# AnimatedRNG/alphazero-rs

Hardware: AMD Instinct MI355X
Metric: selfplay_games_per_sec (higher is better)
Workload: dtype bf16

## Files before the change

alphazero-rs_amd/csrc/az_engine.hip:

```cpp
#include "../../include/az_engine.h"

#include <dlfcn.h>
#include <unistd.h>
#include <rccl/rccl.h>

#include <algorithm>
#include <array>
#include <atomic>
#include <chrono>
#include <cstdio>
#include <cstring>
#include <map>
#include <memory>
#include <mutex>
#include <string>
#include <vector>

#include "az_combine.h"
#include "az_local_comm.h"
#include "az_net.h"
#include "az_train.h"
#include "az_tree.h"

using namespace az;
// ... 767 lines not shown
        return AZ_ERR_HIP;
    }
    *out = e.release();
    return AZ_OK;
}

void az_destroy(az_engine* e) {
    if (!e) return;
    (void)hipSetDevice(e->device);
    (void)hipStreamSynchronize(e->stream);
    (void)az_selfplay_end(e);
    for (auto& kv : e->nets) if (kv.second.conv) convnet_destroy(kv.second.conv);
    for (NetWorkspace* w : e->ws) netws_destroy(w);
    if (e->cache_keys) (void)hipFree(e->cache_keys);
    if (e->cache_pv) (void)hipFree(e->cache_pv);
    if (e->comm && g_rccl.CommDestroy) { (void)g_rccl.CommDestroy(e->comm); e->comm = nullptr; }
    if (e->local) { e->local->leave(e->comm_rank); e->local.reset(); }
    e->tree_pool.clear();
    trainer_destroy(e->trainer);
    { double ms[RG_COUNT] = {0, 0}; e->prof.resolve(ms); }
    (void)hipStreamDestroy(e->stream);
    delete e;
}

const char* az_last_error(const az_engine* e) { return e ? e->err.c_str() : "null engine"; }

az_status az_set_option(az_engine* e, const char* key, int64_t value) {
    if (!e || !key) return AZ_ERR_BAD_ARGUMENT;
    auto is = [&](const char* k) { return std::strcmp(key, k) == 0; };
    if (is("conv2_table") && (value == 0 || value == 1)) { e->netopt.conv2_table = (int)value; return AZ_OK; }
    if (is("conv3_small") && (value == 0 || value == 1)) { e->netopt.conv3_small = (int)value; return AZ_OK; }
    if (is("conv3_tail") && (value == 0 || value == 1)) { e->netopt.conv3_tail = (int)value; return AZ_OK; }
    if (is("ring_packed") && (value == 0 || value == 1)) { e->netopt.ring_packed = (int)value; return AZ_OK; }
    if (is("conv3_planes") && (value == 0 || value == 1)) { e->netopt.conv3_planes = (int)value; return AZ_OK; }
    if (is("narrow_rows") && value >= 0 && value <= 65536) { e->netopt.narrow_rows = (int)value; return AZ_OK; }
    if (is("tree_block4") && (value == 0 || value == 1)) { e->tree_block4 = (int)value; return AZ_OK; }
    if (is("dedup_stats") && (value == 0 || value == 1)) { e->dedup_stats = (int)value; return AZ_OK; }
    if (is("profile_every") && value >= 1 && value <= 1000000) { e->profile_every = (int)value; return AZ_OK; }
    if (is("profile") && (value == 0 || value == 1)) { e->prof.on = value != 0; return AZ_OK; }
    if (is("search_graph") && value >= 0 && value <= 1000 && value % 2 == 0) { e->search_graph = (int)value; return AZ_OK; }
    if (is("search_graph_rows") && value >= 0 && value <= 1000000) { e->search_graph_rows = (int)value; return AZ_OK; }
    if (is("selfplay_async") && (value == 0 || value == 1)) { e->selfplay_async = (int)value; return AZ_OK; }
    if (is("selfplay_async_launches") && value >= 1 && value <= 8) { e->selfplay_async_launches = (int)value; return AZ_OK; }
    if (is("selfplay_async_iters") && value >= 2 && value <= 64) { e->selfplay_async_iters = (int)value; return AZ_OK; }
    if (is("fused_search") && (value == 0 || value == 1)) { e->fused_search = (int)value; return AZ_OK; }
    if (is("eval_dedup") && value >= 0 && value <= 2) { e->eval_dedup = (int)value; return AZ_OK; }
    if (is("eval_cache_log2") && (value == 0 || (value >= 10 && value <= 30))) { e->eval_cache_log2 = (int)value; return AZ_OK; }
    if (is("eval_cache_max_stones") && value >= 0 && value <= 42) { e->eval_cache_max_stones = (int)value; return AZ_OK; }
    if (is("eval_cache_persist") && (value == 0 || value == 1)) { e->eval_cache_persist = (int)value; return AZ_OK; }
    if (is("train_epochs") && value >= 1 && value <= 100000) { e->train_epochs = (int)value; return AZ_OK; }
    if (is("train_batch") && value >= 2 && value <= TRAIN_MAX_BATCH) { e->train_batch = (int)value; return AZ_OK; }
    if (is("train_seed")) { e->train_seed = (uint64_t)value; return AZ_OK; }
    if (is("train_graph") && (value == 0 || value == 1)) { e->train_graph = (int)value; if (e->trainer) trainer_set_graph(e->trainer, value != 0); return AZ_OK; }
    if (is("train_gemm3_ring") && (value == 0 || value == 1)) { e->train_gemm3_ring = (int)value; if (e->trainer) trainer_set_gemm3_ring(e->trainer, value != 0); return AZ_OK; }
    if (is("train_fwd_x3") && (value == 0 || value == 1)) { e->train_fwd_x3 = (int)value; if (e->trainer) trainer_set_fwd_x3(e->trainer, value != 0); return AZ_OK; }
    if (is("train_wgrad_tr") && (value == 0 || value == 1)) { e->train_wgrad_tr = (int)value; if (e->trainer) trainer_set_wgrad_tr(e->trainer, value != 0); return AZ_OK; }
    if (is("train_implicit") && (value == 0 || value == 1)) { e->train_implicit = (int)value; if (e->trainer) trainer_set_implicit(e->trainer, value != 0); return AZ_OK; }
    if (is("train_fork") && (value == 0 || value == 1)) {
        e->train_fork = (int)value;
        if (e->trainer) { (void)hipSetDevice(e->device); trainer_set_fork(e->trainer, value != 0); }
        return AZ_OK;
    }
    if (is("train_gemm") && (value == 0 || value == 1)) { e->train_gemm = (int)value; if (e->trainer) trainer_set_gemm(e->trainer, (int)value); return AZ_OK; }
    if (is("train_fwd_dma") && (value == 0 || value == 1)) { e->train_fwd_dma = (int)value; if (e->trainer) trainer_set_fwd_dma(e->trainer, value != 0); return AZ_OK; }
    if (is("train_lr_e9") && value > 0) { e->hyper.lr = (float)((double)value * 1e-9); return AZ_OK; }
    if (is("train_dropout_e6") && value >= 0 && value < 1000000) { e->hyper.dropout = (float)((double)value * 1e-6); return AZ_OK; }
// ... 1425 lines not shown
```

alphazero-rs_amd/csrc/az_net.h:

```cpp
#pragma once
#include "az_tree.h"

namespace az {

struct ConvNet;
struct NetWorkspace;

struct Layout {
    int C;
    int64_t conv_w[4], conv_b[4], conv_bn[4], fc_w[2], fc_b[2], fc_bn[2], pi_w, pi_b, v_w, v_b, total;
    explicit Layout(int c) : C(c) {
        int64_t o = 0;
        for (int l = 0; l < 4; ++l) {
            int cin = l == 0 ? 2 : C;
            conv_w[l] = o; o += 9ll * cin * C;
            conv_b[l] = o; o += C;
            conv_bn[l] = o; o += 4ll * C;
        }
        const int fin[2] = {6 * C, 1024}, fout[2] = {1024, 512};
        for (int l = 0; l < 2; ++l) {
            fc_w[l] = o; o += (int64_t)fin[l] * fout[l];
            fc_b[l] = o; o += fout[l];
            fc_bn[l] = o; o += 4ll * fout[l];
        }
        pi_w = o; o += 512 * 7; pi_b = o; o += 7;
        v_w = o; o += 512; v_b = o; o += 1;
        total = o;
    }
};


struct NetProfile {
    double conv2_ms = 0, conv2_flops = 0, total_ms = 0, total_flops = 0;
    double conv3_ms = 0, conv3_flops = 0;
    double conv4_ms = 0, conv4_flops = 0;
    double fc_ms = 0, fc_flops = 0;
    double rows = 0;
    double conv2_bytes = 0;
    uint64_t launches = 0;
};

void launch_net_fixture(const EvalBatch& eb, int kind, uint64_t salt, hipStream_t s);

ConvNet* convnet_create(int channels, const char** err);
void convnet_destroy(ConvNet* n);
NetWorkspace* netws_create(int channels, int max_batch, const char** err);
void netws_destroy(NetWorkspace* ws);
int64_t convnet_param_count(int channels);
bool convnet_set_params(ConvNet* n, const float* host_params, int64_t count);
bool convnet_get_params(const ConvNet* n, float* host_params, int64_t count);
void convnet_init_random(ConvNet* n, uint64_t seed);
void netws_resolve_profile(NetWorkspace* ws, NetProfile* prof);
bool netws_conv3_accounting(NetWorkspace* ws, unsigned long long out[2], bool reset);
struct NetOptions {
    int conv2_table = 1;
    int conv3_small = 1;
    int conv3_planes = 1;
    int ring_packed = 1;
    int conv3_tail = 1;
    int narrow_rows = 32;
    int conv3_pp = 0;
    int gemm_variant = 5;
    int conv1_table = 1;
    int conv2_pipe = 1;
    int conv3_pipe = 1;
    int conv3_ring = 0;
    int conv4_big = 0;
    int fc_ring = 1;
    int ring_tile[6] = {0, 0, 0, 0, 0, 0};
};
bool netws_read_clock_stamps(NetWorkspace* ws, unsigned long long* out2048);
bool convnet_prepare(NetWorkspace* ws, const NetOptions& opt);
void convnet_forward(ConvNet* n, NetWorkspace* ws, const EvalBatch& eb, int n_rows_hint, int n_rows_typ, hipStream_t s, NetProfile* prof,
                     const NetOptions& opt);

}
```

alphazero-rs_amd/csrc/az_net.hip:

```cpp
#include "az_net.h"

#include <algorithm>
#include <cmath>
#include <cstring>
#include <vector>

namespace az {

constexpr int ACTIONS = ConnectFour::ACTIONS;

typedef __bf16 bf16x8 __attribute__((ext_vector_type(8)));
typedef float f32x4 __attribute__((ext_vector_type(4)));

__global__ void k_net_fixture(EvalBatch eb, int kind, uint64_t salt) {
    uint32_t i = blockIdx.x * blockDim.x + threadIdx.x;
    if (i >= *eb.n) return;
    float pi[ACTIONS], v;
    if (kind == 0) {
#pragma unroll
        for (int a = 0; a < ACTIONS; ++a) pi[a] = __fdiv_rn(1.0f, 7.0f);
        v = 1.0f;
    } else {
        ulonglong2 s = eb.state[i];
        hashnet_eval(s.x, s.y, salt, pi, &v);
// ... 161 lines not shown
                uint4 o;
                o.x = pack_bf16x2(fmaxf(acc[0] + b0.x, 0.f), fmaxf(acc[1] + b0.y, 0.f));
                o.y = pack_bf16x2(fmaxf(acc[2] + b0.z, 0.f), fmaxf(acc[3] + b0.w, 0.f));
                o.z = pack_bf16x2(fmaxf(acc[4] + b1.x, 0.f), fmaxf(acc[5] + b1.y, 0.f));
                o.w = pack_bf16x2(fmaxf(acc[6] + b1.z, 0.f), fmaxf(acc[7] + b1.w, 0.f));
                *(uint4*)(out + ((size_t)b * 42 + (size_t)(y * 7 + x)) * C + coff) = o;
            }
        }
    }
}

struct GemmDesc {
    const uint16_t* A;
    const uint16_t* W;
    const float* bias;
    uint16_t* out;
    const uint32_t* n_dev;
    int rows_per_sample;
    int out_w;
    int in_h, in_w, in_c;
    int tap_w;
    int cin;
    int K, N;
    int relu;
    unsigned long long* dbg;
    const ulonglong2* states;
    int out_f16;
    int m_min;
    int m_max;
    int m_hi;
    unsigned long long* acct;
    const uint16_t* c3tab;
    const uint16_t* Wp;
    const uint16_t* Wr;
};

constexpr int GBM = 128, GBN = 128, GBK = 64;

template <int LAYER>
__global__ __launch_bounds__(256, 2) void k_gemm_mfma(const GemmDesc d) {
    __shared__ __attribute__((aligned(16))) unsigned char smem[2][(GBM + GBN) * 128];
    const int M = (int)(*d.n_dev) * d.rows_per_sample;
    const int ntaps = d.K / d.cin;
    const int NT = d.N / GBN;
    const int id = blockIdx.x;
    const int xcd = id & 7, j = id >> 3;
    const int ntile = j % NT, mtile = (j / NT) * 8 + xcd;
    const int m0 = mtile * GBM, n0 = ntile * GBN;
    if (m0 >= M) return;
    const int tid = threadIdx.x, lane = tid & 63, wave = tid >> 6;
    const int wr = wave >> 1, wc = wave & 1;
    const int srow = tid >> 3;
    const int chunk = (tid & 7) ^ (srow & 7);
    auto row_off = [&](int q) -> uint32_t {
        int m = m0 + q * 32 + srow;
        m = m < M ? m : M - 1;
        const int b = m / d.rows_per_sample, r = m - b * d.rows_per_sample;
        const int y = r / d.out_w, x = r - y * d.out_w;
        return (uint32_t)(((b * d.in_h + y) * d.in_w + x) * d.in_c + chunk * 8);
    };
    const uint32_t a_off0 = row_off(0), a_off1 = row_off(1), a_off2 = row_off(2), a_off3 = row_off(3);
    const uint32_t b_off0 = (uint32_t)((n0 + srow) * d.K + chunk * 8), b_off1 = b_off0 + 32u * (uint32_t)d.K,
                   b_off2 = b_off0 + 64u * (uint32_t)d.K, b_off3 = b_off0 + 96u * (uint32_t)d.K;
    uint4 ra0, ra1, ra2, ra3, rb0, rb1, rb2, rb3;
#define AZ_GLOAD(kt_)                                                                           \
    {                                                                                           \
// ... 45 lines not shown
        if (kt + 1 < nk) AZ_SWRITE((kt + 1) & 1);
        __syncthreads();
    }
#undef AZ_GLOAD
#undef AZ_SWRITE
#pragma unroll
    for (int nt = 0; nt < 4; ++nt) {
        const int n = n0 + wc * 64 + nt * 16 + fq * 4;
        const float4 bv = d.out_f16 ? make_float4(0.f, 0.f, 0.f, 0.f) : *(const float4*)(d.bias + n);
#pragma unroll
        for (int mt = 0; mt < 4; ++mt) {
            const int m = m0 + wr * 64 + mt * 16 + frow;
            if (m >= M) continue;
            float r0 = acc[mt][nt][0] + bv.x, r1 = acc[mt][nt][1] + bv.y, r2 = acc[mt][nt][2] + bv.z,
                  r3 = acc[mt][nt][3] + bv.w;
            if (d.relu) { r0 = fmaxf(r0, 0.f); r1 = fmaxf(r1, 0.f); r2 = fmaxf(r2, 0.f); r3 = fmaxf(r3, 0.f); }
            uint2 o;
            if (d.out_f16) {
                o.x = pack_f16x2(r0, r1);
                o.y = pack_f16x2(r2, r3);
            } else {
                o.x = pack_bf16x2(r0, r1);
                o.y = pack_bf16x2(r2, r3);
            }
            *(uint2*)(d.out + (size_t)m * d.N + n) = o;
        }
    }
}

__device__ __forceinline__ void lds_dma16(const void* sbase , uint32_t voff, uint32_t lds_addr ) {
    asm volatile("s_mov_b32 m0, %2\n\ts_nop 0\n\tglobal_load_lds_dwordx4 %0, %1" ::"v"(voff), "s"(sbase), "s"(lds_addr) : "memory");
}

template <int NS, int BM>
__device__ __forceinline__ void gemm_ring_body(const GemmDesc& d, unsigned char* smem , const int M) {
    static_assert(BM % 32 == 0 && BM >= 64 && BM <= 192 && NS * (BM * 128 + 16384) <= 163840 && 2 * (BM / 32 + 4) <= 63, "tile");
    constexpr int MT = BM / 32;
    constexpr int STAGE = BM * 128 + 16384;
    constexpr int NDMA = MT + 4;
    const int ntaps = d.K / d.cin;
    const int NT = d.N / GBN;
    const int id = blockIdx.x;
    const int xcd = id & 7, j = id >> 3;
    const int ntile = j % NT, mtile = (j / NT) * 8 + xcd;
    const int m0 = mtile * BM, n0 = ntile * GBN;
    if (m0 >= M) return;
    const int tid = threadIdx.x, lane = tid & 63;
    const int wave = __builtin_amdgcn_readfirstlane(tid >> 6);
    const int wr = wave >> 1, wc = wave & 1;
    const int lrow = lane >> 3;
    const int chunk = (lane & 7) ^ lrow;
    uint32_t a_ob[MT];
#pragma unroll
    for (int q = 0; q < MT; ++q) {
        int m = m0 + (q * 4 + wave) * 8 + lrow;
        m = m < M ? m : M - 1;
        const int b = m / d.rows_per_sample, r = m - b * d.rows_per_sample;
        const int y = r / d.out_w, x = r - y * d.out_w;
        a_ob[q] = (uint32_t)(((b * d.in_h + y) * d.in_w + x) * d.in_c + chunk * 8) * 2u;
    }
    const bool packed = d.Wr != nullptr;
    const uint32_t b_ob = packed ? (uint32_t)(wave * 1024 + lane * 16)
                                 : (uint32_t)((n0 + wave * 8 + lrow) * d.K + chunk * 8) * 2u;
    const size_t w_stride = packed ? (size_t)4096 : (size_t)64 * d.K;
    const char* wr_tile = (const char*)d.Wr + (size_t)ntile * (size_t)(d.K / GBK) * 16384;
    int ks_idx = 0;
    typedef __attribute__((address_space(3))) void* lds_ptr;
    const uint32_t lds0 = (uint32_t)(uintptr_t)(lds_ptr)(smem + wave * 1024);
    int ks_tap = 0, ks_kx = 0;
    uint32_t ks_c0 = 0, ks_toff = 0, ks_kk = 0;
#define AZ_RDMA(buf_)                                                                                   \
    {                                                                                                   \
        const char* abase = (const char*)(d.A + ks_toff);                                               \
        const char* wbase = packed ? wr_tile + (size_t)ks_idx * 16384 : (const char*)(d.W + ks_kk);     \
        ++ks_idx;                                                                                       \
        const uint32_t la = lds0 + (buf_) * STAGE;                                                      \
        _Pragma("unroll") for (int q_ = 0; q_ < MT; ++q_) lds_dma16(abase, a_ob[q_], la + q_ * 4096);   \
        _Pragma("unroll") for (int q_ = 0; q_ < 4; ++q_) lds_dma16(wbase + q_ * w_stride, b_ob, la + BM * 128 + q_ * 4096); \
        ++ks_tap; ++ks_kx; ks_toff += (uint32_t)d.in_c; ks_kk += (uint32_t)d.cin;                       \
        if (ks_kx == d.tap_w) { ks_kx = 0; ks_toff += (uint32_t)((d.in_w - d.tap_w) * d.in_c); }        \
        if (ks_tap == ntaps) { ks_tap = 0; ks_kx = 0; ks_c0 += GBK; ks_toff = ks_c0; ks_kk = ks_c0; }   \
    }
    f32x4 acc[MT][4];
#pragma unroll
    for (int i = 0; i < MT; ++i)
#pragma unroll
        for (int jn = 0; jn < 4; ++jn) acc[i][jn] = f32x4{0.f, 0.f, 0.f, 0.f};
    const int nk = d.K / GBK;
    const int frow = lane & 15, fq = lane >> 4, fsw = lane & 7;
#pragma unroll
    for (int st = 0; st < NS - 1; ++st)
        if (st < nk) AZ_RDMA(st);
    for (int kt = 0; kt < nk; ++kt) {
        const int younger = nk - 1 - kt < NS - 2 ? nk - 1 - kt : NS - 2;
        if (younger >= 2) asm volatile("s_waitcnt vmcnt(%0)" ::"n"(2 * NDMA) : "memory");
        else if (younger == 1) asm volatile("s_waitcnt vmcnt(%0)" ::"n"(NDMA) : "memory");
        else asm volatile("s_waitcnt vmcnt(0)" ::: "memory");
        __builtin_amdgcn_s_barrier();
        __builtin_amdgcn_sched_barrier(0);
        if (kt + NS - 1 < nk) AZ_RDMA((kt + NS - 1) % NS);
        const unsigned char* sA = smem + (kt % NS) * STAGE;
        const unsigned char* sB = sA + BM * 128;
        const int coff0 = ((0 + fq) ^ fsw) << 4, coff1 = ((4 + fq) ^ fsw) << 4;
        bf16x8 fa0[MT], fb0[4], fa1[MT], fb1[4];
#pragma unroll
        for (int mt = 0; mt < MT; ++mt) fa0[mt] = *(const bf16x8*)(sA + (wr * (BM / 2) + mt * 16 + frow) * 128 + coff0);
#pragma unroll
        for (int nt = 0; nt < 4; ++nt) fb0[nt] = *(const bf16x8*)(sB + (wc * 64 + nt * 16 + frow) * 128 + coff0);
#pragma unroll
        for (int mt = 0; mt < MT; ++mt) fa1[mt] = *(const bf16x8*)(sA + (wr * (BM / 2) + mt * 16 + frow) * 128 + coff1);
#pragma unroll
        for (int nt = 0; nt < 4; ++nt) fb1[nt] = *(const bf16x8*)(sB + (wc * 64 + nt * 16 + frow) * 128 + coff1);
#pragma unroll
        for (int mt = 0; mt < MT; ++mt)
#pragma unroll
            for (int nt = 0; nt < 4; ++nt)
                acc[mt][nt] = __builtin_amdgcn_mfma_f32_16x16x32_bf16(fb0[nt], fa0[mt], acc[mt][nt], 0, 0, 0);
#pragma unroll
        for (int mt = 0; mt < MT; ++mt)
#pragma unroll
            for (int nt = 0; nt < 4; ++nt)
                acc[mt][nt] = __builtin_amdgcn_mfma_f32_16x16x32_bf16(fb1[nt], fa1[mt], acc[mt][nt], 0, 0, 0);
        __builtin_amdgcn_sched_group_barrier(0x100, MT + 4, 0);
#pragma unroll
        for (int g = 0; g < MT + 4; ++g) {
            __builtin_amdgcn_sched_group_barrier(0x008, 1, 0);
            __builtin_amdgcn_sched_group_barrier(0x100, 1, 0);
        }
        __builtin_amdgcn_sched_group_barrier(0x008, 8 * MT - (MT + 4), 0);
        __builtin_amdgcn_sched_barrier(0);
    }
#undef AZ_RDMA
    constexpr int EP_STRIDE = 272;
    static_assert(BM * EP_STRIDE <= NS * STAGE, "the output tile must fit the ring");
    __builtin_amdgcn_s_waitcnt(0xC07F);
    __builtin_amdgcn_s_barrier();
#pragma unroll
    for (int nt = 0; nt < 4; ++nt) {
        const int nl = wc * 64 + nt * 16 + fq * 4;
        const float4 bv = *(const float4*)(d.bias + n0 + nl);
#pragma unroll
        for (int mt = 0; mt < MT; ++mt) {
            const int ml = wr * (BM / 2) + mt * 16 + frow;
            float r0 = acc[mt][nt][0] + bv.x, r1 = acc[mt][nt][1] + bv.y, r2 = acc[mt][nt][2] + bv.z,
                  r3 = acc[mt][nt][3] + bv.w;
            if (d.relu) { r0 = fmaxf(r0, 0.f); r1 = fmaxf(r1, 0.f); r2 = fmaxf(r2, 0.f); r3 = fmaxf(r3, 0.f); }
            uint2 o;
            o.x = pack_bf16x2(r0, r1);
            o.y = pack_bf16x2(r2, r3);
            *(uint2*)(smem + ml * EP_STRIDE + nl * 2) = o;
        }
    }
    __syncthreads();
#pragma unroll
    for (int it = 0; it < BM * 16 / 256; ++it) {
        const int idx = it * 256 + tid;
        const int ml = idx >> 4, c = idx & 15;
        const int m = m0 + ml;
        if (m >= M) continue;
        *(uint4*)(d.out + (size_t)m * d.N + n0 + c * 8) = *(const uint4*)(smem + ml * EP_STRIDE + c * 16);
    }
}


AZ_HD int ring_pick_bm(int M, int ncol, int ns, bool conv) {
    auto wgs = [&](int bm) { return (M + bm - 1) / bm * ncol; };
    if (ns == 4) return wgs(64) <= 256 ? 64 : wgs(96) <= 256 ? 96 : 128;
    if (!conv) return wgs(96) <= 512 ? 96 : 128;
    int best = 128;
    float best_cost = 1e30f;
    for (int bm = 96; bm <= 192; bm += 32) {
        const int w = wgs(bm), full = w / 512, rem = w % 512;
        const float cost = (10.f + 0.42f * (float)bm) * ((float)full + (rem == 0 ? 0.f : rem <= 256 ? 0.6f : 1.f));
        if (cost < best_cost) { best_cost = cost; best = bm; }
    }
    return best;
}
template <int LAYER, int NS>
__global__ __launch_bounds__(256, (NS <= 2 ? 2 : 1)) void k_gemm_ring_auto(const GemmDesc d) {
    constexpr int BMAX = NS == 2 ? 192 : 128;
    __shared__ __attribute__((aligned(16))) unsigned char smem[NS * (BMAX * 128 + 16384)];
    const int M = (int)(*d.n_dev) * d.rows_per_sample;
    if (M <= d.m_min || (d.m_hi > 0 && M > d.m_hi)) return;
    const int bm = __builtin_amdgcn_readfirstlane(ring_pick_bm(M, d.N / GBN, NS, d.tap_w > 1));
    if constexpr (NS == 2) {
        if (bm == 96) gemm_ring_body<2, 96>(d, smem, M);
        else if (bm == 160) gemm_ring_body<2, 160>(d, smem, M);
        else if (bm == 192) gemm_ring_body<2, 192>(d, smem, M);
        else gemm_ring_body<2, 128>(d, smem, M);
    } else {
        if (bm == 64) gemm_ring_body<4, 64>(d, smem, M);
        else if (bm == 96) gemm_ring_body<4, 96>(d, smem, M);
        else gemm_ring_body<4, 128>(d, smem, M);
    }
}

[[maybe_unused]] constexpr int HBM_ = 256;
constexpr int HBN_ = 256;


constexpr int IMG_NB = 6, IMG_ROWS = IMG_NB * 42, IMG_ZERO_ROW = 252;


constexpr int HBN2_ = 128;


__device__ __forceinline__ void lds_dma16(const void* sbase, uint32_t voff, uint32_t lds_addr);
template <int LAYER, bool TABLE = false>
__global__ __launch_bounds__(256, 2) void k_conv_same_pipe(const GemmDesc d) {
    __shared__ __attribute__((aligned(16))) unsigned char smem[2 * 32768];
    const int n_boards = (int)(*d.n_dev);
    const int M = n_boards * 42;
    const int C = d.cin;
    const int NT = d.N / HBN2_;
    const int id = blockIdx.x;
    const int xcd = id & 7, j = id >> 3;
    const int ntile = j % NT, mtile = (j / NT) * 8 + xcd;
    const int b0 = mtile * IMG_NB, n0 = ntile * HBN2_;
    if (b0 >= n_boards) return;
    const int tid = threadIdx.x, lane = tid & 63;
    const int wave = __builtin_amdgcn_readfirstlane(tid >> 6);
    const int wr = wave >> 1, wc = wave & 1;
    if (tid < 8) *(uint4*)(smem + IMG_ZERO_ROW * 128 + tid * 16) = make_uint4(0, 0, 0, 0);
// ... 1299 lines not shown
            case 19: hipLaunchKernelGGL((k_conv3_pp<2, 3>), grid, block, 0, s, d); return;
            case 20: hipLaunchKernelGGL((k_conv3_pp<2, 4>), grid, block, 0, s, d); return;
            case 23: hipLaunchKernelGGL((k_conv3_pp<2, 7>), grid, block, 0, s, d); return;
            case 24: hipLaunchKernelGGL((k_conv3_pp<2, 8>), grid, block, 0, s, d); return;
            case 27: hipLaunchKernelGGL((k_conv3_pp<2, 11>), grid, block, 0, s, d); return;
            case 28: hipLaunchKernelGGL((k_conv3_pp<2, 16>), grid, block, 0, s, d); return;
            case 34: hipLaunchKernelGGL((k_conv3_pp<2, 0, 1>), grid, block, 0, s, d); return;
            case 36: hipLaunchKernelGGL((k_conv3_pp<2, 128>), grid, block, 0, s, d); return;
            case 38: hipLaunchKernelGGL((k_conv3_pp<2, 0, 2, 0>), grid, block, 0, s, d); return;
            case 39: hipLaunchKernelGGL((k_conv3_pp<2, 0, 2, 1>), grid, block, 0, s, d); return;
            case 40: hipLaunchKernelGGL((k_conv3_pp<2, 0, 2, 3>), grid, block, 0, s, d); return;
            case 37: hipLaunchKernelGGL((k_conv3_pp<2, 128 + 16>), grid, block, 0, s, d); return;
            case 35: hipLaunchKernelGGL((k_conv3_pp<2, 16, 1>), grid, block, 0, s, d); return;
            case 30: hipLaunchKernelGGL((k_conv3_pp<2, 32>), grid, block, 0, s, d); return;
            case 31: hipLaunchKernelGGL((k_conv3_pp<2, 64>), grid, block, 0, s, d); return;
            case 32: hipLaunchKernelGGL((k_conv3_pp<2, 48>), grid, block, 0, s, d); return;
            case 33: hipLaunchKernelGGL((k_conv3_pp<2, 80>), grid, block, 0, s, d); return;
            case 29: hipLaunchKernelGGL((k_conv3_pp<2, 24>), grid, block, 0, s, d); return;
            default: break;
        }
        hipLaunchKernelGGL((k_conv3_pp<2>), grid, block, 0, s, d);
        return;
    }
#endif
    const int tiles = (rows_hint + C3_NB - 1) / C3_NB;
    const int t8 = (tiles + 7) / 8 * 8;
    const int full_grid = t8 * (d.N / 128);
    if (planes) hipLaunchKernelGGL((k_conv3_auto<2, true>), dim3(full_grid + (tail ? C3_TAIL : 0)), dim3(256), 0, s, d, full_grid, tail ? C3_TAIL : 0);
    else if (tail) hipLaunchKernelGGL((k_conv3_auto<2, false>), dim3(full_grid + C3_TAIL), dim3(256), 0, s, d, full_grid, C3_TAIL);
    else hipLaunchKernelGGL((k_conv_valid_pipe<2, C3_NB, 6, 7, false, 0, true>), dim3(full_grid), dim3(256), 0, s, d);
}

template <int LAYER>
static void launch_ring_auto(const GemmDesc& d, int rows_hint, int rows_typ, hipStream_t s, bool force_one_per_cu = false) {
    const int m_est = (int)((rows_typ > 0 ? (long long)rows_typ * 115 / 100 : (long long)rows_hint) * d.rows_per_sample), ncol = d.N / GBN;
    const bool conv = d.tap_w > 1;
    const int tile_max = conv ? 96 : 128;
    const int m_one = 256 / ncol * tile_max;
    const int m_bound = rows_hint * d.rows_per_sample;
    auto launch = [&](bool one_per_cu, const GemmDesc& dd, int m_cover) {
        const int bmin = one_per_cu ? 64 : 96;
        const int mtb = ((m_cover + bmin - 1) / bmin + 7) / 8 * 8;
        if (one_per_cu) hipLaunchKernelGGL((k_gemm_ring_auto<LAYER, 4>), dim3(mtb * ncol), dim3(256), 0, s, dd);
        else hipLaunchKernelGGL((k_gemm_ring_auto<LAYER, 2>), dim3(mtb * ncol), dim3(256), 0, s, dd);
    };
    if (!force_one_per_cu && !conv && m_bound > m_one && (long long)m_est * 100 >= (long long)m_one * 70 && (long long)m_est * 100 <= (long long)m_one * 140) {
        GemmDesc lo = d, hi = d;
        lo.m_hi = m_one;
        hi.m_min = std::max(d.m_min, m_one);
        launch(true, lo, std::min(m_bound, m_one));
        launch(false, hi, m_bound);
        return;
    }
    const bool one_per_cu = force_one_per_cu || m_bound <= m_one || (m_est + tile_max - 1) / tile_max * ncol <= 256;
    launch(one_per_cu, d, m_bound);
}

#ifdef AZ_DIAG
template <int LAYER>
static bool launch_gemm_diag(const GemmDesc& d, int rows_hint, int rows_typ, hipStream_t s, const NetOptions& o) {
    const int v = o.gemm_variant;
    if ((v == 3 || v == 5) && LAYER == 1 && d.N % HBN_ == 0 && d.cin % 64 == 0) {
        const int tiles = (rows_hint + IMG_NB - 1) / IMG_NB;
        const int t8 = (tiles + 7) / 8 * 8;
        if (v == 5 && o.conv2_pipe) return false;
        if (v == 5 && d.states) hipLaunchKernelGGL((k_conv_img2<LAYER, true>), dim3(t8 * (d.N / HBN2_)), dim3(256), 0, s, d);
        else if (v == 5) hipLaunchKernelGGL((k_conv_img2<LAYER>), dim3(t8 * (d.N / HBN2_)), dim3(256), 0, s, d);
        else hipLaunchKernelGGL((k_conv_img<LAYER>), dim3(t8 * (d.N / HBN_)), dim3(512), 0, s, d);
        return true;
    }
    const bool big = v >= 1 && (LAYER == 1 || LAYER == 2 || (LAYER == 3 && !o.ring_tile[3] && (o.conv4_big == 1 || (o.conv4_big == 2 && rows_typ >= 4096)))) &&
                     d.N % HBN_ == 0;
    if constexpr (LAYER == 2) if (v == 5 && o.conv3_ring) {
        const int mt = (rows_hint * d.rows_per_sample + GBM - 1) / GBM;
        const int mt8 = (mt + 7) / 8 * 8;
        if (o.conv3_ring == 3) launch_ring_auto<LAYER>(d, rows_hint, rows_typ, s, true);
        else if (o.conv3_ring == 2) hipLaunchKernelGGL((k_gemm_ring<LAYER, 4>), dim3(mt8 * (d.N / GBN)), dim3(256), 0, s, d);
        else hipLaunchKernelGGL((k_gemm_ring<LAYER, 2>), dim3(mt8 * (d.N / GBN)), dim3(256), 0, s, d);
        return true;
    }
    if constexpr (LAYER == 2) if (v == 5 && d.rows_per_sample == 20) {
        if ((o.conv3_small && conv3_is_small(d, rows_hint, rows_typ)) || o.conv3_pipe == 1) return false;
        const int tiles = (rows_hint + C3_NB - 1) / C3_NB;
        const int t8 = (tiles + 7) / 8 * 8;
        const dim3 g3(t8 * (d.N / 128)), b3(256);
        switch (o.conv3_pipe) {
            case 2: hipLaunchKernelGGL((k_conv_valid_pipe<LAYER, C3_NB, 6, 7, false, 0, false>), g3, b3, 0, s, d); break;
            case 3: hipLaunchKernelGGL((k_conv_valid_pipe<LAYER, C3_NB, 6, 7, true, 0, true>), g3, b3, 0, s, d); break;
            case 10: hipLaunchKernelGGL((k_conv_valid_pipe<LAYER, C3_NB, 6, 7, false, -1, true>), g3, b3, 0, s, d); break;
            case 9: hipLaunchKernelGGL((k_conv_valid_pipe<LAYER, C3_NB, 6, 7, false, -2, true>), g3, b3, 0, s, d); break;
            case 11: hipLaunchKernelGGL((k_conv_valid_pipe<LAYER, C3_NB, 6, 7, false, 1, true>), g3, b3, 0, s, d); break;
            case 12: hipLaunchKernelGGL((k_conv_valid_pipe<LAYER, C3_NB, 6, 7, false, 2, true>), g3, b3, 0, s, d); break;
            case 13: hipLaunchKernelGGL((k_conv_valid_pipe<LAYER, C3_NB, 6, 7, false, 3, true>), g3, b3, 0, s, d); break;
            case 14: hipLaunchKernelGGL((k_conv_valid_pipe<LAYER, C3_NB, 6, 7, false, 4, true>), g3, b3, 0, s, d); break;
            case 15: hipLaunchKernelGGL((k_conv_valid_pipe<LAYER, C3_NB, 6, 7, false, 5, true>), g3, b3, 0, s, d); break;
            default: hipLaunchKernelGGL((k_conv_valid_img2<LAYER, C3_NB, 6, 7, 2>), g3, b3, 0, s, d); break;
        }
        return true;
    }
    if (v == 5 && !big && o.fc_ring == 1 && !(LAYER >= 3 && o.ring_tile[LAYER])) return false;
    if (big) {
        const int mt = (rows_hint * d.rows_per_sample + HBM_ - 1) / HBM_;
        const int mt8 = (mt + 7) / 8 * 8;
        const dim3 grid(mt8 * (d.N / HBN_)), block(512);
        if (v == 1) hipLaunchKernelGGL((k_gemm256<LAYER, 0>), grid, block, 0, s, d);
        else if (v == 11) hipLaunchKernelGGL((k_gemm256<LAYER, 1, 1>), grid, block, 0, s, d);
        else if (v == 12) hipLaunchKernelGGL((k_gemm256<LAYER, 1, 2>), grid, block, 0, s, d);
        else if (v == 13) hipLaunchKernelGGL((k_gemm256<LAYER, 1, 3>), grid, block, 0, s, d);
        else if (v == 14) hipLaunchKernelGGL((k_gemm256<LAYER, 1, 4>), grid, block, 0, s, d);
        else if (v == 15) hipLaunchKernelGGL((k_gemm256<LAYER, 1, 5>), grid, block, 0, s, d);
        else if (v == 16) hipLaunchKernelGGL((k_gemm256<LAYER, 1, 6>), grid, block, 0, s, d);
        else if (v == 17) hipLaunchKernelGGL((k_gemm256<LAYER, 1, 7>), grid, block, 0, s, d);
        else hipLaunchKernelGGL((k_gemm256<LAYER, 1>), grid, block, 0, s, d);
        return true;
    }
    const int mt = (rows_hint * d.rows_per_sample + GBM - 1) / GBM;
    const int mt8 = (mt + 7) / 8 * 8;
    const int grid = mt8 * (d.N / GBN);
    if (v == 5 && o.fc_ring) {
        auto ring = [&](auto bm_c, auto ns_c) {
            constexpr int BM = decltype(bm_c)::value, NS = decltype(ns_c)::value;
            const int mtb = ((rows_hint * d.rows_per_sample + BM - 1) / BM + 7) / 8 * 8;
            hipLaunchKernelGGL((k_gemm_ring<LAYER, NS, BM>), dim3(mtb * (d.N / GBN)), dim3(256), 0, s, d);
        };
        using std::integral_constant;
        if constexpr (LAYER >= 3) {
            switch (o.ring_tile[LAYER]) {
                case 642: ring(integral_constant<int, 64>{}, integral_constant<int, 2>{}); return true;
                case 644: ring(integral_constant<int, 64>{}, integral_constant<int, 4>{}); return true;
                case 962: ring(integral_constant<int, 96>{}, integral_constant<int, 2>{}); return true;
                case 964: ring(integral_constant<int, 96>{}, integral_constant<int, 4>{}); return true;
                case 1282: ring(integral_constant<int, 128>{}, integral_constant<int, 2>{}); return true;
                case 1284: ring(integral_constant<int, 128>{}, integral_constant<int, 4>{}); return true;
                case 1602: ring(integral_constant<int, 160>{}, integral_constant<int, 2>{}); return true;
                case 1922: ring(integral_constant<int, 192>{}, integral_constant<int, 2>{}); return true;
                default: break;
            }
        }
        if (o.fc_ring == 2) {
            const int m_typ = (rows_typ > 0 ? rows_typ : rows_hint) * d.rows_per_sample, ncol = d.N / GBN;
            const bool conv = d.tap_w > 1;
            const int ns = (m_typ + (conv ? 95 : 127)) / (conv ? 96 : 128) * ncol <= 256 ? 4 : 2;
            switch (ring_pick_bm(m_typ, ncol, ns, conv) * 10 + ns) {
                case 644: ring(integral_constant<int, 64>{}, integral_constant<int, 4>{}); break;
                case 964: ring(integral_constant<int, 96>{}, integral_constant<int, 4>{}); break;
                case 1284: ring(integral_constant<int, 128>{}, integral_constant<int, 4>{}); break;
                case 962: ring(integral_constant<int, 96>{}, integral_constant<int, 2>{}); break;
                case 1602: ring(integral_constant<int, 160>{}, integral_constant<int, 2>{}); break;
                case 1922: ring(integral_constant<int, 192>{}, integral_constant<int, 2>{}); break;
                default: ring(integral_constant<int, 128>{}, integral_constant<int, 2>{}); break;
            }
            return true;
        }
        if (o.fc_ring == 1) return false;
        hipLaunchKernelGGL((k_gemm_ring<LAYER, 2>), dim3(grid), dim3(256), 0, s, d);
        return true;
    }
    hipLaunchKernelGGL(k_gemm_mfma<LAYER>, dim3(grid), dim3(256), 0, s, d);
    return true;
}
#endif

template <int LAYER>
static void launch_gemm(const GemmDesc& d, int rows_hint, int rows_typ, hipStream_t s, const NetOptions& o) {
#ifdef AZ_DIAG
    if (launch_gemm_diag<LAYER>(d, rows_hint, rows_typ, s, o)) return;
#endif
    GemmDesc dd = d;
    if constexpr (LAYER >= 2) if (o.narrow_rows > 0 && d.N % 32 == 0) {
        const int lim = o.narrow_rows * (LAYER == 2 ? 1 : LAYER == 3 ? 2 : 4);
        const int est = rows_typ > 0 ? rows_typ : rows_hint;
        if (est <= 16 * lim) {
            dd.m_max = lim * d.rows_per_sample;
            const int rows_cov = rows_hint < lim ? rows_hint : lim;
            const dim3 grid((unsigned)skinny_waves_max(rows_cov * d.rows_per_sample, d.N)), block(64);
            const int nk = d.K / GBK;
            if (nk % 8 == 0) hipLaunchKernelGGL((k_gemm_skinny<LAYER, 8>), grid, block, 0, s, dd);
            else if (nk % 6 == 0) hipLaunchKernelGGL((k_gemm_skinny<LAYER, 6>), grid, block, 0, s, dd);
            else hipLaunchKernelGGL((k_gemm_skinny<LAYER, 2>), grid, block, 0, s, dd);
            if (rows_hint <= lim) return;
            dd.m_min = dd.m_max;
        }
    }
    const GemmDesc& d2 = dd;
    if constexpr (LAYER == 1) if (d.N % HBN_ == 0 && d.cin % 64 == 0) {
        if (d.states) launch_conv2_gemm<true>(d2, rows_hint, s);
        else launch_conv2_gemm<false>(d2, rows_hint, s);
        return;
    }
    if constexpr (LAYER == 2) {
        if (o.conv3_small && conv3_is_small(d2, rows_hint, rows_typ)) launch_ring_auto<LAYER>(d2, rows_hint, rows_typ, s, true);
        else launch_conv3_image(d2, rows_hint, s, o.conv3_tail != 0, o.conv3_planes != 0, o.conv3_pp);
        return;
    }

    launch_ring_auto<LAYER>(d2, rows_hint, rows_typ, s);
}

static hipEvent_t net_event(NetWorkspace* n) {
    if (!n->ev_pool.empty()) { hipEvent_t e = n->ev_pool.back(); n->ev_pool.pop_back(); return e; }
    hipEvent_t e = nullptr;
    (void)hipEventCreate(&e);
    return e;
}

bool netws_conv3_accounting(NetWorkspace* n, unsigned long long out[2], bool reset) {
    if (!n || !n->acct) return true;
    unsigned long long h[2] = {0, 0};
    if (hipMemcpy(h, n->acct, sizeof h, hipMemcpyDeviceToHost) != hipSuccess) return false;
    out[0] += h[0]; out[1] += h[1];
    return !reset || hipMemset(n->acct, 0, sizeof h) == hipSuccess;
}

void netws_resolve_profile(NetWorkspace* n, NetProfile* prof) {
    if (!n) return;
    const int C = n->C;
    const double f_conv = 2.0 * 9.0 * C * C;
    const double per_sample = 2.0 * (42.0 * 18 * C) + f_conv * (42 + 20 + 6) + 2.0 * (6.0 * C * 1024 + 1024.0 * 512 + 512.0 * 8);
    if (!n->open.empty() && hipMemcpy(n->pinned_n, n->d_nlog, (size_t)n->pinned_next * sizeof(uint32_t), hipMemcpyDeviceToHost) != hipSuccess)
        prof = nullptr;
    for (auto& r : n->open) {
        float conv2 = 0, conv3 = 0, conv4 = 0, fcs = 0, total = 0;
        if (hipEventElapsedTime(&conv2, r.e1, r.e2) == hipSuccess && hipEventElapsedTime(&conv3, r.e2, r.e2b) == hipSuccess &&
            hipEventElapsedTime(&conv4, r.e2b, r.e2c) == hipSuccess && hipEventElapsedTime(&fcs, r.e2c, r.e3) == hipSuccess &&
            hipEventElapsedTime(&total, r.e0, r.e3) == hipSuccess && prof) {
            const double rows = (double)*r.n;
            prof->conv2_ms += conv2;
            prof->conv3_ms += conv3;
            prof->conv3_flops += f_conv * 20.0 * rows;
// ... 108 lines not shown
```

alphazero-rs_amd/csrc/az_net_diag.inc:

```

typedef _Float16 f16x8 __attribute__((ext_vector_type(8)));
__global__ __launch_bounds__(256) void k_conv2_table(const EvalBatch eb, const uint16_t* __restrict__ U ,
                                                     const float* __restrict__ bias , uint16_t* __restrict__ out ,
                                                     int C) {
    extern __shared__ __attribute__((aligned(16))) unsigned char u0_lds[];
    for (int i = threadIdx.x; i < 9 * C / 8; i += blockDim.x) ((uint4*)u0_lds)[i] = ((const uint4*)U)[i];
    __syncthreads();
    const int lane = threadIdx.x & 63;
    const uint32_t items = *eb.n * 6u;
    const uint32_t wave0 = blockIdx.x * 4u + (threadIdx.x >> 6), nwaves = gridDim.x * 4u;
    const int cg = C / 8;
    for (uint32_t it = wave0; it < items; it += nwaves) {
        const uint32_t b = it / 6u;
        const int y = (int)(it - b * 6u);
        const ulonglong2 sv = eb.state[b];
        const int ly = y - 1 + (lane < 21 ? lane / 7 : 0), lx = lane < 21 ? lane % 7 : 0;
        const uint32_t mypat = (ly >= 0 && ly < 6) ? conv1_pattern(sv.x, sv.y, ly, lx) : 0u;
        for (int x = 0; x < 7; ++x) {
            uint32_t row[9];
#pragma unroll
            for (int t = 0; t < 9; ++t) {
                const int ky = t / 3, qy = y + ky - 1, qx = x + t % 3 - 1;
                const bool in = qy >= 0 && qy < 6 && qx >= 0 && qx < 7;
                const uint32_t pq = (uint32_t)__builtin_amdgcn_readlane((int)mypat, in ? ky * 7 + qx : 0);
                row[t] = in ? pq * 9u + (uint32_t)t : 0xFFFFFFFFu;
            }
            for (int c8 = lane; c8 < cg; c8 += 64) {
                f16x8 u[9];
#pragma unroll
                for (int t = 0; t < 9; ++t) {
                    if (row[t] == 0xFFFFFFFFu) continue;
                    if (row[t] < 9u) u[t] = *(const f16x8*)(u0_lds + ((size_t)row[t] * C + (size_t)c8 * 8) * 2);
                    else u[t] = *(const f16x8*)(U + ((size_t)row[t] * C + (size_t)c8 * 8));
                }
                float acc[8] = {0.f, 0.f, 0.f, 0.f, 0.f, 0.f, 0.f, 0.f};
#pragma unroll
                for (int t = 0; t < 9; ++t)
                    if (row[t] != 0xFFFFFFFFu) {
#pragma unroll
                        for (int i = 0; i < 8; ++i) acc[i] += (float)u[t][i];
                    }
                const float4 b0 = *(const float4*)(bias + c8 * 8), b1 = *(const float4*)(bias + c8 * 8 + 4);
                uint4 o;
                o.x = pack_bf16x2(fmaxf(acc[0] + b0.x, 0.f), fmaxf(acc[1] + b0.y, 0.f));
                o.y = pack_bf16x2(fmaxf(acc[2] + b0.z, 0.f), fmaxf(acc[3] + b0.w, 0.f));
                o.z = pack_bf16x2(fmaxf(acc[4] + b1.x, 0.f), fmaxf(acc[5] + b1.y, 0.f));
                o.w = pack_bf16x2(fmaxf(acc[6] + b1.z, 0.f), fmaxf(acc[7] + b1.w, 0.f));
                *(uint4*)(out + ((size_t)b * 42 + (size_t)(y * 7 + x)) * C + (size_t)c8 * 8) = o;
            }
        }
    }
}

template <int LAYER, int NS, int BM = 128>
__global__ __launch_bounds__(256, (NS <= 2 ? 2 : 1)) void k_gemm_ring(const GemmDesc d) {
    __shared__ __attribute__((aligned(16))) unsigned char smem[NS * (BM * 128 + 16384)];
    gemm_ring_body<NS, BM>(d, smem, (int)(*d.n_dev) * d.rows_per_sample);
}

template <int LAYER, int PIPE, int ABLATE = 0>
__global__ __launch_bounds__(512, 2) void k_gemm256(const GemmDesc d) {
    __shared__ __attribute__((aligned(16))) unsigned char smem[2 * (HBM_ + HBN_) * 128];
    const int M = (int)(*d.n_dev) * d.rows_per_sample;
    const int ntaps = d.K / d.cin;
    const int NT = d.N / HBN_;
    const int id = blockIdx.x;
    const int xcd = id & 7, j = id >> 3;
    const int ntile = j % NT, mtile = (j / NT) * 8 + xcd;
    const int m0 = mtile * HBM_, n0 = ntile * HBN_;
    if (m0 >= M) return;
    const int tid = threadIdx.x, lane = tid & 63;
    const int wave = __builtin_amdgcn_readfirstlane(tid >> 6);
    const int wr = wave >> 2, wc = wave & 3;
    const int lrow = lane >> 3;
    const int chunk = (lane & 7) ^ lrow;
    auto row_off = [&](int q) -> uint32_t {
        int m = m0 + (q * 8 + wave) * 8 + lrow;
        m = m < M ? m : M - 1;
        const int b = m / d.rows_per_sample, r = m - b * d.rows_per_sample;
        const int y = r / d.out_w, x = r - y * d.out_w;
        return (uint32_t)(((b * d.in_h + y) * d.in_w + x) * d.in_c + chunk * 8);
    };
    const uint32_t a_off0 = row_off(0), a_off1 = row_off(1), a_off2 = row_off(2), a_off3 = row_off(3);
    const uint32_t b_off0 = (uint32_t)((n0 + wave * 8 + lrow) * d.K + chunk * 8);
    const uint32_t b_step = 64u * (uint32_t)d.K;
    const uint32_t a_ob0 = a_off0 * 2u, a_ob1 = a_off1 * 2u, a_ob2 = a_off2 * 2u, a_ob3 = a_off3 * 2u;
    const uint32_t b_ob0 = b_off0 * 2u, b_ob1 = (b_off0 + b_step) * 2u, b_ob2 = (b_off0 + 2u * b_step) * 2u,
                   b_ob3 = (b_off0 + 3u * b_step) * 2u;
    typedef __attribute__((address_space(3))) void* lds_ptr;
    typedef const __attribute__((address_space(1))) void* gbl_ptr;
// ... 605 lines not shown
```

Baseline: 10100.

## Add 64-column ring GEMM tiles for FC layers and tighter grid sizing

Templates the ring GEMM body on tile width BN so the FC layers can use 64-column tiles (BM 64 or 96) when that keeps the workgroup count within 256. For small batches this spreads the FC GEMMs over more workgroups. Grid size is now computed from the actual tile choice, and with fc_one_launch the split into two launches is used in a narrower band of batch sizes. Narrower tiles reuse each A tile across fewer columns and add device-side dispatch branches. Diagnostic options are added to describe the chosen tiles.

Result: no change. 10060 (median of 2 runs) (-0.4%).

```diff
diff --git a/alphazero-rs_amd/csrc/az_engine.hip b/alphazero-rs_amd/csrc/az_engine.hip
--- a/alphazero-rs_amd/csrc/az_engine.hip
+++ b/alphazero-rs_amd/csrc/az_engine.hip
@@ -823,6 +823,9 @@
     if (is("conv3_small") && (value == 0 || value == 1)) { e->netopt.conv3_small = (int)value; return AZ_OK; }
     if (is("conv3_tail") && (value == 0 || value == 1)) { e->netopt.conv3_tail = (int)value; return AZ_OK; }
     if (is("ring_packed") && (value == 0 || value == 1)) { e->netopt.ring_packed = (int)value; return AZ_OK; }
+    if (is("fc_cols") && (value == 0 || value == 1)) { e->netopt.fc_cols = (int)value; return AZ_OK; }
+    if (is("fc_one_launch") && (value == 0 || value == 1)) { e->netopt.fc_one_launch = (int)value; return AZ_OK; }
+    if (is("describe_fc_tiles") && (value == 4 || value == 5)) { e->err = convnet_fc_tiles((int)value, e->cfg.max_batch, e->netopt); return AZ_OK; }
     if (is("conv3_planes") && (value == 0 || value == 1)) { e->netopt.conv3_planes = (int)value; return AZ_OK; }
     if (is("narrow_rows") && value >= 0 && value <= 65536) { e->netopt.narrow_rows = (int)value; return AZ_OK; }
     if (is("tree_block4") && (value == 0 || value == 1)) { e->tree_block4 = (int)value; return AZ_OK; }
diff --git a/alphazero-rs_amd/csrc/az_net.h b/alphazero-rs_amd/csrc/az_net.h
--- a/alphazero-rs_amd/csrc/az_net.h
+++ b/alphazero-rs_amd/csrc/az_net.h
@@ -1,5 +1,6 @@
 #pragma once
 #include "az_tree.h"
+#include <string>
 
 namespace az {
 
@@ -59,6 +60,8 @@
     int ring_packed = 1;
     int conv3_tail = 1;
     int narrow_rows = 32;
+    int fc_cols = 1;
+    int fc_one_launch = 1;
     int conv3_pp = 0;
     int gemm_variant = 5;
     int conv1_table = 1;
@@ -69,6 +72,7 @@
     int fc_ring = 1;
     int ring_tile[6] = {0, 0, 0, 0, 0, 0};
 };
+std::string convnet_fc_tiles(int layer, int max_rows, const NetOptions& opt);
 bool netws_read_clock_stamps(NetWorkspace* ws, unsigned long long* out2048);
 bool convnet_prepare(NetWorkspace* ws, const NetOptions& opt);
 void convnet_forward(ConvNet* n, NetWorkspace* ws, const EvalBatch& eb, int n_rows_hint, int n_rows_typ, hipStream_t s, NetProfile* prof,
diff --git a/alphazero-rs_amd/csrc/az_net.hip b/alphazero-rs_amd/csrc/az_net.hip
--- a/alphazero-rs_amd/csrc/az_net.hip
+++ b/alphazero-rs_amd/csrc/az_net.hip
@@ -217,6 +217,7 @@
     unsigned long long* acct;
     const uint16_t* c3tab;
     const uint16_t* Wp;
+    int cols64;
     const uint16_t* Wr;
 };
 
@@ -328,18 +329,19 @@
     asm volatile("s_mov_b32 m0, %2\n\ts_nop 0\n\tglobal_load_lds_dwordx4 %0, %1" ::"v"(voff), "s"(sbase), "s"(lds_addr) : "memory");
 }
 
-template <int NS, int BM>
+template <int NS, int BM, int BN = GBN>
 __device__ __forceinline__ void gemm_ring_body(const GemmDesc& d, unsigned char* smem , const int M) {
-    static_assert(BM % 32 == 0 && BM >= 64 && BM <= 192 && NS * (BM * 128 + 16384) <= 163840 && 2 * (BM / 32 + 4) <= 63, "tile");
+    static_assert(BM % 32 == 0 && BM >= 64 && BM <= 192 && (BN == 64 || BN == 128) && NS * (BM + BN) * 128 <= 163840 && 2 * (BM / 32 + BN / 32) <= 63, "tile");
     constexpr int MT = BM / 32;
-    constexpr int STAGE = BM * 128 + 16384;
-    constexpr int NDMA = MT + 4;
+    constexpr int NTW = BN / 32;
+    constexpr int STAGE = (BM + BN) * 128;
+    constexpr int NDMA = MT + NTW;
     const int ntaps = d.K / d.cin;
-    const int NT = d.N / GBN;
+    const int NT = d.N / BN;
     const int id = blockIdx.x;
     const int xcd = id & 7, j = id >> 3;
     const int ntile = j % NT, mtile = (j / NT) * 8 + xcd;
-    const int m0 = mtile * BM, n0 = ntile * GBN;
+    const int m0 = mtile * BM, n0 = ntile * BN;
     if (m0 >= M) return;
     const int tid = threadIdx.x, lane = tid & 63;
     const int wave = __builtin_amdgcn_readfirstlane(tid >> 6);
@@ -359,7 +361,7 @@
     const uint32_t b_ob = packed ? (uint32_t)(wave * 1024 + lane * 16)
                                  : (uint32_t)((n0 + wave * 8 + lrow) * d.K + chunk * 8) * 2u;
     const size_t w_stride = packed ? (size_t)4096 : (size_t)64 * d.K;
-    const char* wr_tile = (const char*)d.Wr + (size_t)ntile * (size_t)(d.K / GBK) * 16384;
+    const char* wr_tile = (const char*)d.Wr + (size_t)(n0 / GBN) * (size_t)(d.K / GBK) * 16384 + (n0 % GBN) * 128;
     int ks_idx = 0;
     typedef __attribute__((address_space(3))) void* lds_ptr;
     const uint32_t lds0 = (uint32_t)(uintptr_t)(lds_ptr)(smem + wave * 1024);
@@ -372,16 +374,16 @@
         ++ks_idx;                                                                                       \
         const uint32_t la = lds0 + (buf_) * STAGE;                                                      \
         _Pragma("unroll") for (int q_ = 0; q_ < MT; ++q_) lds_dma16(abase, a_ob[q_], la + q_ * 4096);   \
-        _Pragma("unroll") for (int q_ = 0; q_ < 4; ++q_) lds_dma16(wbase + q_ * w_stride, b_ob, la + BM * 128 + q_ * 4096); \
+        _Pragma("unroll") for (int q_ = 0; q_ < NTW; ++q_) lds_dma16(wbase + q_ * w_stride, b_ob, la + BM * 128 + q_ * 4096); \
         ++ks_tap; ++ks_kx; ks_toff += (uint32_t)d.in_c; ks_kk += (uint32_t)d.cin;                       \
         if (ks_kx == d.tap_w) { ks_kx = 0; ks_toff += (uint32_t)((d.in_w - d.tap_w) * d.in_c); }        \
         if (ks_tap == ntaps) { ks_tap = 0; ks_kx = 0; ks_c0 += GBK; ks_toff = ks_c0; ks_kk = ks_c0; }   \
     }
-    f32x4 acc[MT][4];
+    f32x4 acc[MT][NTW];
 #pragma unroll
     for (int i = 0; i < MT; ++i)
 #pragma unroll
-        for (int jn = 0; jn < 4; ++jn) acc[i][jn] = f32x4{0.f, 0.f, 0.f, 0.f};
+        for (int jn = 0; jn < NTW; ++jn) acc[i][jn] = f32x4{0.f, 0.f, 0.f, 0.f};
     const int nk = d.K / GBK;
     const int frow = lane & 15, fq = lane >> 4, fsw = lane & 7;
 #pragma unroll
@@ -398,42 +400,42 @@
         const unsigned char* sA = smem + (kt % NS) * STAGE;
         const unsigned char* sB = sA + BM * 128;
         const int coff0 = ((0 + fq) ^ fsw) << 4, coff1 = ((4 + fq) ^ fsw) << 4;
-        bf16x8 fa0[MT], fb0[4], fa1[MT], fb1[4];
+        bf16x8 fa0[MT], fb0[NTW], fa1[MT], fb1[NTW];
 #pragma unroll
         for (int mt = 0; mt < MT; ++mt) fa0[mt] = *(const bf16x8*)(sA + (wr * (BM / 2) + mt * 16 + frow) * 128 + coff0);
 #pragma unroll
-        for (int nt = 0; nt < 4; ++nt) fb0[nt] = *(const bf16x8*)(sB + (wc * 64 + nt * 16 + frow) * 128 + coff0);
+        for (int nt = 0; nt < NTW; ++nt) fb0[nt] = *(const bf16x8*)(sB + (wc * (BN / 2) + nt * 16 + frow) * 128 + coff0);
 #pragma unroll
         for (int mt = 0; mt < MT; ++mt) fa1[mt] = *(const bf16x8*)(sA + (wr * (BM / 2) + mt * 16 + frow) * 128 + coff1);
 #pragma unroll
-        for (int nt = 0; nt < 4; ++nt) fb1[nt] = *(const bf16x8*)(sB + (wc * 64 + nt * 16 + frow) * 128 + coff1);
+        for (int nt = 0; nt < NTW; ++nt) fb1[nt] = *(const bf16x8*)(sB + (wc * (BN / 2) + nt * 16 + frow) * 128 + coff1);
 #pragma unroll
         for (int mt = 0; mt < MT; ++mt)
 #pragma unroll
-            for (int nt = 0; nt < 4; ++nt)
+            for (int nt = 0; nt < NTW; ++nt)
                 acc[mt][nt] = __builtin_amdgcn_mfma_f32_16x16x32_bf16(fb0[nt], fa0[mt], acc[mt][nt], 0, 0, 0);
 #pragma unroll
         for (int mt = 0; mt < MT; ++mt)
 #pragma unroll
-            for (int nt = 0; nt < 4; ++nt)
+            for (int nt = 0; nt < NTW; ++nt)
                 acc[mt][nt] = __builtin_amdgcn_mfma_f32_16x16x32_bf16(fb1[nt], fa1[mt], acc[mt][nt], 0, 0, 0);
-        __builtin_amdgcn_sched_group_barrier(0x100, MT + 4, 0);
-#pragma unroll
-        for (int g = 0; g < MT + 4; ++g) {
+        __builtin_amdgcn_sched_group_barrier(0x100, MT + NTW, 0);
+#pragma unroll
+        for (int g = 0; g < MT + NTW; ++g) {
             __builtin_amdgcn_sched_group_barrier(0x008, 1, 0);
             __builtin_amdgcn_sched_group_barrier(0x100, 1, 0);
         }
-        __builtin_amdgcn_sched_group_barrier(0x008, 8 * MT - (MT + 4), 0);
+        __builtin_amdgcn_sched_group_barrier(0x008, 2 * MT * NTW - (MT + NTW), 0);
         __builtin_amdgcn_sched_barrier(0);
     }
 #undef AZ_RDMA
-    constexpr int EP_STRIDE = 272;
+    constexpr int EP_STRIDE = BN * 2 + 16;
     static_assert(BM * EP_STRIDE <= NS * STAGE, "the output tile must fit the ring");
     __builtin_amdgcn_s_waitcnt(0xC07F);
     __builtin_amdgcn_s_barrier();
 #pragma unroll
-    for (int nt = 0; nt < 4; ++nt) {
-        const int nl = wc * 64 + nt * 16 + fq * 4;
+    for (int nt = 0; nt < NTW; ++nt) {
+        const int nl = wc * (BN / 2) + nt * 16 + fq * 4;
         const float4 bv = *(const float4*)(d.bias + n0 + nl);
 #pragma unroll
         for (int mt = 0; mt < MT; ++mt) {
@@ -448,10 +450,11 @@
         }
     }
     __syncthreads();
-#pragma unroll
-    for (int it = 0; it < BM * 16 / 256; ++it) {
+    constexpr int EPC = BN / 8;
+#pragma unroll
+    for (int it = 0; it < BM * EPC / 256; ++it) {
         const int idx = it * 256 + tid;
-        const int ml = idx >> 4, c = idx & 15;
+        const int ml = idx / EPC, c = idx % EPC;
         const int m = m0 + ml;
         if (m >= M) continue;
         *(uint4*)(d.out + (size_t)m * d.N + n0 + c * 8) = *(const uint4*)(smem + ml * EP_STRIDE + c * 16);
@@ -472,19 +475,40 @@
     }
     return best;
 }
+AZ_HD int ring_pick_tile(int M, int ncol, int ns, bool conv, bool cols64) {
+    if (cols64 && ns == 4 && !conv) {
+        auto wgs = [&](int bm, int per128) { return (M + bm - 1) / bm * ncol * per128; };
+        if (wgs(64, 2) <= 256) return 64 * 1000 + 64;
+        if (wgs(96, 2) <= 256) return 96 * 1000 + 64;
+    }
+    return ring_pick_bm(M, ncol, ns, conv) * 1000 + GBN;
+}
+static int ring_grid(int m_cover, int ncol, int ns, bool cols64) {
+    int grid = 0;
+    for (int m = 32; m < m_cover + 32; m += 32) {
+        const int mm = std::min(m, m_cover), t = ring_pick_tile(mm, ncol, ns, false, cols64), bm = t / 1000, bn = t % 1000;
+        grid = std::max(grid, ((mm + bm - 1) / bm + 7) / 8 * 8 * (ncol * (GBN / bn)));
+    }
+    return grid;
+}
 template <int LAYER, int NS>
 __global__ __launch_bounds__(256, (NS <= 2 ? 2 : 1)) void k_gemm_ring_auto(const GemmDesc d) {
     constexpr int BMAX = NS == 2 ? 192 : 128;
     __shared__ __attribute__((aligned(16))) unsigned char smem[NS * (BMAX * 128 + 16384)];
     const int M = (int)(*d.n_dev) * d.rows_per_sample;
     if (M <= d.m_min || (d.m_hi > 0 && M > d.m_hi)) return;
-    const int bm = __builtin_amdgcn_readfirstlane(ring_pick_bm(M, d.N / GBN, NS, d.tap_w > 1));
+    const int tile = __builtin_amdgcn_readfirstlane(ring_pick_tile(M, d.N / GBN, NS, d.tap_w > 1, d.cols64 != 0));
+    const int bm = tile / 1000;
     if constexpr (NS == 2) {
         if (bm == 96) gemm_ring_body<2, 96>(d, smem, M);
         else if (bm == 160) gemm_ring_body<2, 160>(d, smem, M);
         else if (bm == 192) gemm_ring_body<2, 192>(d, smem, M);
         else gemm_ring_body<2, 128>(d, smem, M);
     } else {
+        if constexpr (LAYER >= 4) {
+            if (tile == 64 * 1000 + 64) return gemm_ring_body<4, 64, 64>(d, smem, M);
+            if (tile == 96 * 1000 + 64) return gemm_ring_body<4, 96, 64>(d, smem, M);
+        }
         if (bm == 64) gemm_ring_body<4, 64>(d, smem, M);
         else if (bm == 96) gemm_ring_body<4, 96>(d, smem, M);
         else gemm_ring_body<4, 128>(d, smem, M);
@@ -1850,7 +1874,11 @@
 }
 
 template <int LAYER>
-static void launch_ring_auto(const GemmDesc& d, int rows_hint, int rows_typ, hipStream_t s, bool force_one_per_cu = false) {
+static void launch_ring_auto(const GemmDesc& d0, int rows_hint, int rows_typ, hipStream_t s, const NetOptions& o, bool force_one_per_cu = false) {
+    GemmDesc d = d0;
+    const bool fc = LAYER >= 4 && d.tap_w == 1;
+    d.cols64 = fc && o.fc_cols ? 1 : 0;
+    const bool tight = fc && o.fc_one_launch;
     const int m_est = (int)((rows_typ > 0 ? (long long)rows_typ * 115 / 100 : (long long)rows_hint) * d.rows_per_sample), ncol = d.N / GBN;
     const bool conv = d.tap_w > 1;
     const int tile_max = conv ? 96 : 128;
@@ -1859,10 +1887,13 @@
     auto launch = [&](bool one_per_cu, const GemmDesc& dd, int m_cover) {
         const int bmin = one_per_cu ? 64 : 96;
         const int mtb = ((m_cover + bmin - 1) / bmin + 7) / 8 * 8;
-        if (one_per_cu) hipLaunchKernelGGL((k_gemm_ring_auto<LAYER, 4>), dim3(mtb * ncol), dim3(256), 0, s, dd);
-        else hipLaunchKernelGGL((k_gemm_ring_auto<LAYER, 2>), dim3(mtb * ncol), dim3(256), 0, s, dd);
+        int grid = mtb * ncol;
+        if (tight) grid = ring_grid(m_cover, ncol, one_per_cu ? 4 : 2, dd.cols64 != 0);
+        else if (dd.cols64) grid = std::max(grid, ring_grid(m_cover, ncol, one_per_cu ? 4 : 2, true));
+        if (one_per_cu) hipLaunchKernelGGL((k_gemm_ring_auto<LAYER, 4>), dim3(grid), dim3(256), 0, s, dd);
+        else hipLaunchKernelGGL((k_gemm_ring_auto<LAYER, 2>), dim3(grid), dim3(256), 0, s, dd);
     };
-    if (!force_one_per_cu && !conv && m_bound > m_one && (long long)m_est * 100 >= (long long)m_one * 70 && (long long)m_est * 100 <= (long long)m_one * 140) {
+    if (!force_one_per_cu && !conv && m_bound > m_one && (long long)m_est * 100 >= (long long)m_one * (tight ? 90 : 70) && (long long)m_est * 100 <= (long long)m_one * 140) {
         GemmDesc lo = d, hi = d;
         lo.m_hi = m_one;
         hi.m_min = std::max(d.m_min, m_one);
@@ -1892,7 +1923,7 @@
     if constexpr (LAYER == 2) if (v == 5 && o.conv3_ring) {
         const int mt = (rows_hint * d.rows_per_sample + GBM - 1) / GBM;
         const int mt8 = (mt + 7) / 8 * 8;
-        if (o.conv3_ring == 3) launch_ring_auto<LAYER>(d, rows_hint, rows_typ, s, true);
+        if (o.conv3_ring == 3) launch_ring_auto<LAYER>(d, rows_hint, rows_typ, s, o, true);
         else if (o.conv3_ring == 2) hipLaunchKernelGGL((k_gemm_ring<LAYER, 4>), dim3(mt8 * (d.N / GBN)), dim3(256), 0, s, d);
         else hipLaunchKernelGGL((k_gemm_ring<LAYER, 2>), dim3(mt8 * (d.N / GBN)), dim3(256), 0, s, d);
         return true;
@@ -1942,6 +1973,19 @@
             hipLaunchKernelGGL((k_gemm_ring<LAYER, NS, BM>), dim3(mtb * (d.N / GBN)), dim3(256), 0, s, d);
         };
         using std::integral_constant;
+        if constexpr (LAYER >= 4) {
+            auto ring64 = [&](auto bm_c) {
+                constexpr int BM = decltype(bm_c)::value;
+                const int mtb = ((rows_hint * d.rows_per_sample + BM - 1) / BM + 7) / 8 * 8;
+                hipLaunchKernelGGL((k_gemm_ring<LAYER, 4, BM, 64>), dim3(mtb * (d.N / 64)), dim3(256), 0, s, d);
+            };
+            switch (o.ring_tile[LAYER]) {
+                case 5644: ring64(integral_constant<int, 64>{}); return true;
+                case 5964: ring64(integral_constant<int, 96>{}); return true;
+                case 6284: ring64(integral_constant<int, 128>{}); return true;
+                default: break;
+            }
+        }
         if constexpr (LAYER >= 3) {
             switch (o.ring_tile[LAYER]) {
                 case 642: ring(integral_constant<int, 64>{}, integral_constant<int, 2>{}); return true;
@@ -1978,6 +2022,18 @@
     return true;
 }
 #endif
+
+std::string convnet_fc_tiles(int layer, int max_rows, const NetOptions& o) {
+    const int ncol = (layer == 4 ? 1024 : 512) / GBN;
+    std::string out = "skinny:" + std::to_string(o.narrow_rows * 4) + " line:" + std::to_string(256 / ncol * 128);
+    for (int ns = 4; ns >= 2; ns -= 2)
+        for (int m = 1, prev = 0; m <= max_rows; ++m) {
+            const int t = ring_pick_tile(m, ncol, ns, false, o.fc_cols != 0);
+            if (t != prev) out += " " + std::to_string(ns) + ":" + std::to_string(m) + ":" + std::to_string(t / 1000) + ":" + std::to_string(t % 1000);
+            prev = t;
+        }
+    return out;
+}
 
 template <int LAYER>
 static void launch_gemm(const GemmDesc& d, int rows_hint, int rows_typ, hipStream_t s, const NetOptions& o) {
@@ -2007,12 +2063,12 @@
         return;
     }
     if constexpr (LAYER == 2) {
-        if (o.conv3_small && conv3_is_small(d2, rows_hint, rows_typ)) launch_ring_auto<LAYER>(d2, rows_hint, rows_typ, s, true);
+        if (o.conv3_small && conv3_is_small(d2, rows_hint, rows_typ)) launch_ring_auto<LAYER>(d2, rows_hint, rows_typ, s, o, true);
         else launch_conv3_image(d2, rows_hint, s, o.conv3_tail != 0, o.conv3_planes != 0, o.conv3_pp);
         return;
     }
 
-    launch_ring_auto<LAYER>(d2, rows_hint, rows_typ, s);
+    launch_ring_auto<LAYER>(d2, rows_hint, rows_typ, s, o);
 }
 
 static hipEvent_t net_event(NetWorkspace* n) {
diff --git a/alphazero-rs_amd/csrc/az_net_diag.inc b/alphazero-rs_amd/csrc/az_net_diag.inc
--- a/alphazero-rs_amd/csrc/az_net_diag.inc
+++ b/alphazero-rs_amd/csrc/az_net_diag.inc
@@ -52,10 +52,10 @@
     }
 }
 
-template <int LAYER, int NS, int BM = 128>
+template <int LAYER, int NS, int BM = 128, int BN = GBN>
 __global__ __launch_bounds__(256, (NS <= 2 ? 2 : 1)) void k_gemm_ring(const GemmDesc d) {
-    __shared__ __attribute__((aligned(16))) unsigned char smem[NS * (BM * 128 + 16384)];
-    gemm_ring_body<NS, BM>(d, smem, (int)(*d.n_dev) * d.rows_per_sample);
+    __shared__ __attribute__((aligned(16))) unsigned char smem[NS * (BM + BN) * 128];
+    gemm_ring_body<NS, BM, BN>(d, smem, (int)(*d.n_dev) * d.rows_per_sample);
 }
 
 template <int LAYER, int PIPE, int ABLATE = 0>
```
